# ShengkaiWu/IoU-aware-single-stage-object-detector

Hardware: AMD Instinct MI355X
Metric: images/sec at 1333x800, IoU-aware RetinaNet R-50-FPN (higher is better)
Workload: dtype fp32; 1 GPU; IoU-aware RetinaNet R-50-FPN fp32, batch 8 per GPU, 3x800x1344 (1333x800 padded to /32), random-init weights, whole inference path incl. NMS, device-to-host copy and bbox2result (the reference's simple_test: per-class arrays on the host; batch i's host part runs under batch i+1's device part, the last one inside the timed region); global_batch=8, parallelism=dp1, dets_per_image=100

## Files before the change

### include/iouaware.h

```cpp
#ifndef IOUAWARE_H
#define IOUAWARE_H

#include <stddef.h>
#include <stdint.h>

#ifdef __cplusplus
extern "C" {
#endif

#define IA_MAX_LEVELS 8
#define IA_MAX_ANCHORS 16
#define IA_MAX_NMS_PRE 4096
#define IA_MAX_CANDIDATES 8192
#define IA_MAX_PER_IMG 1024

#define IA_F32 0
#define IA_BF16 1
#define IA_F16 2
#define IA_F64 3

#define IA_LAYOUT_NCHW 0
#define IA_LAYOUT_NHWC 1

#define IA_CLS_SIGMOID 0
// ... 88 lines not shown
                           int batch, int R, int C, float score_thr, float iou_thr,
                           int max_per_img, int candidates, void *workspace,
                           size_t workspace_bytes, float *dets, int32_t *labels, int32_t *rows,
                           int32_t *num, void *stream);

int ia_decode_stage(const ia_head_geom *g, const ia_level_ptrs *p, int batch, int dtype,
                    const float *img_hw, const float *scale_factor, int rescale, void *workspace,
                    size_t workspace_bytes, void *stream);

int ia_get_bboxes_workspace_layout(const ia_head_geom *g, int batch, size_t offsets[8]);

size_t ia_nms_workspace_bytes(int n);
int ia_nms(const float *dets, int n, float iou_thr, int32_t *keep, int32_t *count, void *workspace,
           size_t workspace_bytes, void *stream);

size_t ia_nms_f64_workspace_bytes(int n);
int ia_nms_f64(const double *dets, int n, float iou_thr, int32_t *keep, int32_t *count,
               void *workspace, size_t workspace_bytes, void *stream);

int ia_soft_nms(const float *dets, int n, float iou_thr, int method, float sigma, float min_score,
                float *out_dets, int32_t *out_inds, int32_t *count, void *stream);

typedef struct {
    const uint8_t *src;
    int32_t src_h, src_w, dst_h, dst_w, flip;
} ia_image_desc;
int ia_image_transform(const ia_image_desc *imgs, int batch, const float *mean, const float *std,
                       int to_rgb, int pad_h, int pad_w, int channels_last, float *out,
                       void *stream);

typedef struct {
    int32_t num_levels, batch;
    int32_t H[IA_MAX_LEVELS], W[IA_MAX_LEVELS];
} ia_wino_geom;
typedef struct {
    int32_t c0, n;
    int32_t dst_channels, dst_offset;
    float *dst[IA_MAX_LEVELS];
} ia_wino_seg;
int ia_wino_tiles(const ia_wino_geom *g, int32_t *tiles);
int ia_wino_input_transform(const ia_wino_geom *g, const float *const *x, int channels, int groups,
                            const float *pre_scale, const float *pre_shift, int pre_relu, float *V,
                            void *stream);
int ia_wino_output_transform(const ia_wino_geom *g, const float *M, int channels, int groups,
                             const float *bias, int relu, int nseg, const ia_wino_seg *segs,
                             void *stream);
int ia_wino_mid_transform(const ia_wino_geom *g, const float *M, int channels, int groups_m,
                          const float *bias, int relu, float *V, int groups_v, void *stream);
int ia_wino_in_gemm(const ia_wino_geom *g, const float *const *x, int channels, const float *pre_scale,
                    const float *pre_shift, int pre_relu, const float *u_packed, float *M, void *stream);
int ia_wino_conv3x3_c64(const ia_wino_geom *g, const float *const *x, int channels, const float *pre_scale,
                        const float *pre_shift, int pre_relu, const float *u_packed, const float *bias,
                        int relu, float *const *y, void *stream);

int ia_wino_grad_output_transform(const ia_wino_geom *g, const float *const *dy, int channels,
                                  float *dM, void *stream);

#define IA_COLSUM_MAX_STRIPS 512
size_t ia_relu_bwd_bias_grad_workspace_bytes(int64_t rows, int n);
int ia_wino_weight_transform(const float *w, int n_in, int n_out, int64_t stride_in,
                             int64_t stride_out, int64_t stride_ky, int64_t stride_kx, int flip,
                             const double *G, float *U, void *stream);
int ia_wino_weight_grad(const float *dU, int n_in, int n_out, const double *G, float *dW,
                        int64_t stride_in, int64_t stride_out, int64_t stride_ky, int64_t stride_kx,
                        void *stream);
int ia_bn_fold_fwd(const float *w, const float *gamma, const float *beta, const float *mean,
                   const float *inv_std, int cout, int K, float *w_out, float *b_out, void *stream);
int ia_bn_fold_bwd(const float *dw_folded, const float *db_folded, const float *w, const float *gamma,
                   const float *mean, const float *inv_std, int cout, int K, float *dw,
                   float *dgamma, float *dbeta, void *stream);
int ia_relu_bwd_bias_grad(const float *dy, const float *y, int64_t rows, int n, float *g, float *db,
                          void *workspace, size_t workspace_bytes, void *stream);

int ia_linear_bias_act(const float *A, const float *W, const float *bias, const float *residual,
                       float *D, int64_t rows, int k, int n, int relu, void *workspace,
                       size_t workspace_bytes, void *stream);
int ia_linear_bias_act_bf16(const void *A, const void *W, const float *bias, const void *residual,
                            void *D, int64_t rows, int k, int n, int relu, void *workspace,
                            size_t workspace_bytes, void *stream);
int ia_batched_gemm(const float *A, const float *W, float *D, int batch, int64_t rows, int k, int n,
                    void *workspace, size_t workspace_bytes, void *stream);
int ia_batched_gemm_stream(const float *A, const float *W, float *D, int batch, int64_t rows, int k,
                           int n, void *stream);

size_t ia_im2col3x3_bytes(int B, int H, int W, int C, int stride, int dtype);
int ia_im2col3x3_nhwc(const void *x, void *col, int B, int H, int W, int C, int stride, int dtype,
                      void *stream);
int ia_conv1x1_strided(const void *x, const void *W_kn, const float *bias, const void *residual,
                       void *D, int B, int H, int W, int k, int n, int stride, int relu, int dtype,
                       void *workspace, size_t workspace_bytes, void *stream);
int ia_col2im3x3_nhwc(const void *dcol, void *dx, int B, int H, int W, int C, int stride, int dtype,
                      void *stream);

size_t ia_deform_im2col3x3_bytes(int B, int H, int W, int C, int stride, int pad, int dil);
int ia_deform_im2col3x3_nhwc(const float *x, const float *offset, int64_t offset_pix_stride,
                             const float *mask, int64_t mask_pix_stride, int mask_logits,
                             float *col, int B, int H, int W, int C, int stride, int pad,
                             int dil, int deformable_groups, void *stream);
int ia_deform_col2im3x3_nhwc(const float *dcol, const float *x, const float *offset,
                             int64_t offset_pix_stride, const float *mask,
                             int64_t mask_pix_stride, float *dx, float *d_offset, float *d_mask,
                             int B, int H, int W, int C, int stride, int pad, int dil,
                             int deformable_groups, void *stream);

int ia_gemm_tuning(int mode);

// ... 416 lines not shown
```

### iou-aware-single-stage-object-detector_amd/csrc/wino.hip

```cpp
#include <string.h>
#include "ia_internal.hpp"
#include "ia_wino.hpp"

namespace ia {

typedef float f32x4_t __attribute__((ext_vector_type(4)));
__device__ __forceinline__ float4 load_nt(const float *p)
{
    const f32x4_t q = __builtin_nontemporal_load(reinterpret_cast<const f32x4_t *>(p));
    return make_float4(q.x, q.y, q.z, q.w);
}
__device__ __forceinline__ void store_nt(float *p, const float4 &v)
{
    f32x4_t q; q.x = v.x; q.y = v.y; q.z = v.z; q.w = v.w;
    __builtin_nontemporal_store(q, reinterpret_cast<f32x4_t *>(p));
}
__device__ __forceinline__ float4 f4(float v) { return make_float4(v, v, v, v); }
__device__ __forceinline__ float4 operator+(const float4 &a, const float4 &b) { return make_float4(a.x + b.x, a.y + b.y, a.z + b.z, a.w + b.w); }
__device__ __forceinline__ float4 operator-(const float4 &a, const float4 &b) { return make_float4(a.x - b.x, a.y - b.y, a.z - b.z, a.w - b.w); }
__device__ __forceinline__ float4 operator*(float s, const float4 &a) { return make_float4(s * a.x, s * a.y, s * a.z, s * a.w); }

__device__ __forceinline__ void bt6(const float4 (&d)[6], float4 (&o)[6])
{
    o[0] = (4.0f * d[0] - 5.0f * d[2]) + d[4];
// ... 559 lines not shown
#pragma unroll
            for (int i = 0; i < 4; ++i) {
                float4 o[4];
                at6(s[i], o);
                const int y = 4 * tyi + i, ly = ly0 + i;
#pragma unroll
                for (int j = 0; j < 4; ++j) {
                    const int xx = 4 * txi + j, lx = lx0 + j;
                    float4 v = o[j] + bz;
                    if (a.relu) v = make_float4(v.x > 0.f ? v.x : 0.f, v.y > 0.f ? v.y : 0.f,
                                                v.z > 0.f ? v.z : 0.f, v.w > 0.f ? v.w : 0.f);
                    v = (y < H && xx < W) ? v : f4(0.0f);
                    if (ly >= 0 && ly < kMidP && lx >= 0 && lx < kMidP)
                        *reinterpret_cast<float4 *>(sy + (ly * kMidP + lx) * kMidCh) = v;
                }
            }
        } else {
#pragma unroll
            for (int i = 0; i < 4; ++i)
#pragma unroll
                for (int j = 0; j < 4; ++j) {
                    const int ly = ly0 + i, lx = lx0 + j;
                    if (ly >= 0 && ly < kMidP && lx >= 0 && lx < kMidP)
                        *reinterpret_cast<float4 *>(sy + (ly * kMidP + lx) * kMidCh) = f4(0.0f);
                }
        }
    }
    __syncthreads();

    const int tl = tid / kMidQ, tyl = tl / kMidB, txl = tl - tyl * kMidB;
    const int tyi = kMidB * byi + tyl, txi = kMidB * bxi + txl;
    if (tyi >= ty_n || txi >= tx) return;
    const float *sp = s_y + ((4 * tyl) * kMidP + 4 * txl) * kMidCh + cq;
    float4 tmp[6][6];
#pragma unroll
    for (int j = 0; j < 6; ++j) {
        float4 col[6], o[6];
#pragma unroll
        for (int i = 0; i < 6; ++i) col[i] = *reinterpret_cast<const float4 *>(sp + (i * kMidP + j) * kMidCh);
        bt6(col, o);
#pragma unroll
        for (int i = 0; i < 6; ++i) tmp[i][j] = o[i];
        __builtin_amdgcn_sched_barrier(0);
    }
    float *v = a.V + (size_t)gv * 36 * vstride + (size_t)(tbase + tyi * tx + txi) * a.Cv + (c - gv * a.Cv);
#pragma unroll
    for (int i = 0; i < 6; ++i) {
        float4 o[6];
        bt6(tmp[i], o);
#pragma unroll
        for (int j = 0; j < 6; ++j)
            *reinterpret_cast<float4 *>(v + (size_t)(i * 6 + j) * vstride) = o[j];
    }
}

}

extern "C" {

int ia_wino_tiles(const ia_wino_geom *g, int32_t *tiles)
{
    ia::WinoLevels w;
    int rc = ia::make_wino_levels(g, w);
    if (rc) return rc;
    if (tiles) *tiles = w.tile_off[w.L];
    return 0;
}

int ia_wino_input_transform(const ia_wino_geom *g, const float *const *x, int channels, int groups,
                            const float *pre_scale, const float *pre_shift, int pre_relu, float *V,
                            void *stream)
{
    ia::WinoInArgs a;
    int rc = ia::make_wino_levels(g, a.lv);
    if (rc) return rc;
    if (!x || !V || channels < 4 || (channels & 3) || groups < 1 || channels % groups) return IA_E_ARG;
    a.Ctot = channels; a.Cg = channels / groups; a.T = a.lv.tile_off[a.lv.L];
    if (a.Cg & 3) return IA_E_ARG;
    for (int l = 0; l < IA_MAX_LEVELS; ++l) {
        a.x[l] = (l < a.lv.L) ? x[l] : nullptr;
        if (l < a.lv.L && (!x[l] || ((uintptr_t)x[l] & 15u))) return IA_E_ARG;
    }
    a.V = V;
    if (pre_scale && !pre_shift) return IA_E_ARG;
    a.pre_scale = pre_scale; a.pre_shift = pre_shift; a.pre_relu = pre_relu ? 1 : 0;
    a.tpw = ia::tiles_per_wave(channels);
    const int waves = (a.T + a.tpw - 1) / a.tpw;
    dim3 grid((unsigned)((waves + 7) / 8 * 8), (unsigned)((channels / 4 + 63) / 64));
    if (a.tpw > 1) hipLaunchKernelGGL(ia::k_wino_in<true>, grid, dim3(64), 0, (hipStream_t)stream, a);
    else hipLaunchKernelGGL(ia::k_wino_in<false>, grid, dim3(64), 0, (hipStream_t)stream, a);
    return ia::hip_status(hipGetLastError());
}

int ia_wino_in_gemm(const ia_wino_geom *g, const float *const *x, int channels, const float *pre_scale,
                    const float *pre_shift, int pre_relu, const float *u_packed, float *M, void *stream)
{
    ia::WinoInGemmArgs a;
    int rc = ia::make_wino_levels(g, a.lv);
    if (rc) return rc;
    if (!x || !u_packed || !M || channels != 64) return IA_E_ARG;
    if (((uintptr_t)u_packed & 15u) || ((uintptr_t)M & 15u) || ((uintptr_t)pre_scale & 15u) ||
        ((uintptr_t)pre_shift & 15u))
        return IA_E_ARG;
    for (int l = 0; l < IA_MAX_LEVELS; ++l) {
        a.x[l] = (l < a.lv.L) ? x[l] : nullptr;
        if (l < a.lv.L && (!x[l] || ((uintptr_t)x[l] & 15u))) return IA_E_ARG;
// ... 73 lines not shown
    a.T = a.lv.tile_off[a.lv.L]; a.relu = relu ? 1 : 0; a.nseg = nseg;
    memset(a.seg, 0, sizeof(a.seg));
    for (int k = 0; k < nseg; ++k) {
        const ia_wino_seg &s = segs[k];
        if (s.c0 < 0 || s.n < 1 || s.c0 + s.n > channels || s.dst_channels < s.n + s.dst_offset ||
            s.dst_offset < 0)
            return IA_E_ARG;
        if (k > 0 && s.c0 < segs[k - 1].c0 + segs[k - 1].n) return IA_E_ARG;
        a.seg[k].c0 = s.c0; a.seg[k].n = s.n; a.seg[k].Cdst = s.dst_channels; a.seg[k].coff = s.dst_offset;
        for (int l = 0; l < a.lv.L; ++l) {
            if (!s.dst[l]) return IA_E_ARG;
            a.seg[k].dst[l] = s.dst[l];
        }
    }
    a.tpw = ia::tiles_per_wave(channels);
    const int waves = (a.T + a.tpw - 1) / a.tpw;
    dim3 grid((unsigned)((waves + 7) / 8 * 8), (unsigned)((channels / 4 + 63) / 64));
    if (a.tpw > 1) hipLaunchKernelGGL(ia::k_wino_out<true>, grid, dim3(64), 0, (hipStream_t)stream, a);
    else hipLaunchKernelGGL(ia::k_wino_out<false>, grid, dim3(64), 0, (hipStream_t)stream, a);
    return ia::hip_status(hipGetLastError());
}

int ia_wino_mid_transform(const ia_wino_geom *g, const float *M, int channels, int groups_m,
                          const float *bias, int relu, float *V, int groups_v, void *stream)
{
    ia::WinoMidArgs a;
    int rc = ia::make_wino_levels(g, a.lv);
    if (rc) return rc;
    if (!M || !V || channels < ia::kMidCh || groups_m < 1 || channels % groups_m || groups_v < 1 ||
        channels % groups_v)
        return IA_E_ARG;
    a.M = M; a.bias = bias; a.V = V; a.Ctot = channels;
    a.Cm = channels / groups_m; a.Cv = channels / groups_v;
    if (a.Cm % ia::kMidCh || a.Cv % ia::kMidCh || ((uintptr_t)M & 15u) || ((uintptr_t)V & 15u) ||
        ((uintptr_t)bias & 15u))
        return IA_E_ARG;
    a.T = a.lv.tile_off[a.lv.L]; a.relu = relu ? 1 : 0;
    int64_t n = 0;
    for (int l = 0; l < IA_MAX_LEVELS; ++l) {
        const bool on = l < a.lv.L;
        const int ty = on ? a.lv.tpi[l] / a.lv.tx[l] : 0;
        a.bx[l] = on ? (a.lv.tx[l] + ia::kMidB - 1) / ia::kMidB : 0;
        a.bpi[l] = on ? ((ty + ia::kMidB - 1) / ia::kMidB) * a.bx[l] : 0;
        a.blk_off[l] = (int32_t)n;
        n += (int64_t)a.lv.B * a.bpi[l];
    }
    a.blk_off[IA_MAX_LEVELS] = (int32_t)n;
    a.nblk = (int32_t)n;
    dim3 grid((unsigned)((n + 7) / 8 * 8), (unsigned)(channels / ia::kMidCh));
    hipLaunchKernelGGL(ia::k_wino_mid, grid, dim3(ia::kMidThreads), 0, (hipStream_t)stream, a);
    return ia::hip_status(hipGetLastError());
}

}
```

### iou-aware-single-stage-object-detector_amd/iouaware/_lib.py

```python
import ctypes as C
import os

IA_MAX_LEVELS = 8
IA_MAX_ANCHORS = 16
IA_MAX_NMS_PRE = 4096
IA_MAX_CANDIDATES = 8192
IA_MAX_PER_IMG = 1024
IA_F32, IA_BF16, IA_F16, IA_F64 = 0, 1, 2, 3
IA_LAYOUT_NCHW, IA_LAYOUT_NHWC = 0, 1
IA_CLS_SIGMOID, IA_CLS_SOFTMAX = 0, 1
IA_CLS_SIGMOID_NOIOU, IA_CLS_SOFTMAX_NOIOU = 2, 3
IA_LOSS_SLOTS = 64
IA_MAX_TARGET_BATCH = 16
IA_GN_CHUNK = 256

_CSRC = os.path.join(os.path.dirname(os.path.abspath(__file__)), '..', 'csrc')
SO_PATH = os.path.abspath(os.path.join(_CSRC, 'libiouaware_hip.so'))


class HeadGeom(C.Structure):
    _fields_ = [('num_levels', C.c_int32), ('num_anchors', C.c_int32),
                ('num_classes', C.c_int32), ('nms_pre', C.c_int32),
                ('H', C.c_int32 * IA_MAX_LEVELS), ('W', C.c_int32 * IA_MAX_LEVELS),
                ('stride', C.c_int32 * IA_MAX_LEVELS),
# ... 105 lines not shown
SIGNATURES = {
    'ia_version': (C.c_char_p, []),
    'ia_geom_sizes': (_i, [_G, C.POINTER(C.c_int32), C.POINTER(C.c_int32), C.POINTER(C.c_int32)]),
    'ia_decode_fuse_rowmax': (_i, [_G, _P, _i, _i, _vp, _vp]),
    'ia_select_topk_workspace_bytes': (_sz, [_G, _i]),
    'ia_select_topk': (_i, [_G, _vp, _i, _vp, _vp, _sz, _vp]),
    'ia_decode_fuse_rowmax_grouped': (_i, [_G, _P, _i, _i, _vp, _vp, _sz, _vp]),
    'ia_select_topk_grouped': (_i, [_G, _vp, _i, _vp, _vp, _sz, _vp]),
    'ia_decode_stage': (_i, [_G, _P, _i, _i, _vp, _vp, _i, _vp, _sz, _vp]),
    'ia_get_bboxes_status_offset': (_sz, [_G, _i]),
    'ia_debug_fused_spin_limit': (_i, [_i64]),
    'ia_profile_stage_events': (_i, [_vp, _vp]),
    'ia_gather_decode': (_i, [_G, _P, _i, _i, _vp, _vp, _vp, _i, _vp, _vp, _vp, _vp]),
    'ia_multiclass_nms_workspace_bytes': (_sz, [_i, _i, _i]),
    'ia_multiclass_nms': (_i, [_vp, _vp, _vp, _i, _i, _i, _f, _f, _i, _vp, _sz, _vp, _vp, _vp,
                               _vp, _vp, _vp, _vp]),
    'ia_multiclass_soft_nms_workspace_bytes': (_sz, [_i, _i, _i]),
    'ia_multiclass_soft_nms': (_i, [_vp, _vp, _i, _i, _i, _f, _f, _i, _f, _f, _i, _vp, _sz, _vp, _vp,
                                    _vp, _vp, _vp, _vp, _vp]),
    'ia_soft_nms': (_i, [_vp, _i, _f, _i, _f, _f, _vp, _vp, _vp, _vp]),
    'ia_get_bboxes_workspace_bytes': (_sz, [_G, _i]),
    'ia_get_bboxes': (_i, [_G, _P, _i, _i, _vp, _vp, _i, _f, _f, _i, _vp, _sz, _vp, _vp, _vp,
                           _vp, _vp]),
    'ia_multiclass_nms_lazy_workspace_bytes': (_sz, [_i, _i, _i]),
    'ia_multiclass_nms_lazy': (_i, [_vp, _vp, _vp, _i, _i, _i, _f, _f, _i, _i, _vp, _sz, _vp, _vp, _vp,
                                    _vp, _vp]),
    'ia_get_bboxes_lazy': (_i, [_G, _P, _i, _i, _vp, _vp, _i, _f, _f, _i, _i, _vp, _sz, _vp, _vp, _vp,
                                _vp, _vp]),
    'ia_get_bboxes_workspace_layout': (_i, [_G, _i, C.POINTER(_sz * 8)]),
    'ia_nms_workspace_bytes': (_sz, [_i]),
    'ia_nms': (_i, [_vp, _i, _f, _vp, _vp, _vp, _sz, _vp]),
    'ia_nms_f64_workspace_bytes': (_sz, [_i]),
    'ia_nms_f64': (_i, [_vp, _i, _f, _vp, _vp, _vp, _sz, _vp]),
    'ia_image_transform': (_i, [C.POINTER(ImageDesc), _i, C.POINTER(C.c_float), C.POINTER(C.c_float),
                                _i, _i, _i, _i, _vp, _vp]),
    'ia_wino_tiles': (_i, [C.POINTER(WinoGeom), C.POINTER(C.c_int32)]),
    'ia_wino_input_transform': (_i, [C.POINTER(WinoGeom), C.POINTER(C.c_void_p), _i, _i, _vp, _vp, _i,
                                     _vp, _vp]),
    'ia_wino_grad_output_transform': (_i, [C.POINTER(WinoGeom), C.POINTER(C.c_void_p), _i, _vp, _vp]),
    'ia_wino_weight_transform': (_i, [_vp, _i, _i, C.c_int64, C.c_int64, C.c_int64, C.c_int64, _i,
                                      C.POINTER(C.c_double), _vp, _vp]),
    'ia_wino_weight_grad': (_i, [_vp, _i, _i, C.POINTER(C.c_double), _vp, C.c_int64, C.c_int64,
                                 C.c_int64, C.c_int64, _vp]),
    'ia_bn_fold_fwd': (_i, [_vp, _vp, _vp, _vp, _vp, _i, _i, _vp, _vp, _vp]),
    'ia_bn_fold_bwd': (_i, [_vp, _vp, _vp, _vp, _vp, _vp, _i, _i, _vp, _vp, _vp, _vp]),
    'ia_relu_bwd_bias_grad_workspace_bytes': (C.c_size_t, [C.c_int64, _i]),
    'ia_relu_bwd_bias_grad': (_i, [_vp, _vp, C.c_int64, _i, _vp, _vp, _vp, C.c_size_t, _vp]),
    'ia_wino_output_transform': (_i, [C.POINTER(WinoGeom), _vp, _i, _i, _vp, _i, _i,
                                      C.POINTER(WinoSeg), _vp]),
    'ia_wino_mid_transform': (_i, [C.POINTER(WinoGeom), _vp, _i, _i, _vp, _i, _vp, _i, _vp]),
    'ia_wino_in_gemm': (_i, [C.POINTER(WinoGeom), C.POINTER(C.c_void_p), _i, _vp, _vp, _i, _vp, _vp, _vp]),
    'ia_wino_conv3x3_c64': (_i, [C.POINTER(WinoGeom), C.POINTER(C.c_void_p), _i, _vp, _vp, _i, _vp, _vp, _i,
                                 C.POINTER(C.c_void_p), _vp]),
    'ia_linear_bias_act': (_i, [_vp, _vp, _vp, _vp, _vp, _i64, _i, _i, _i, _vp, _sz, _vp]),
    'ia_linear_bias_act_bf16': (_i, [_vp, _vp, _vp, _vp, _vp, _i64, _i, _i, _i, _vp, _sz, _vp]),
    'ia_batched_gemm': (_i, [_vp, _vp, _vp, _i, _i64, _i, _i, _vp, _sz, _vp]),
    'ia_batched_gemm_stream': (_i, [_vp, _vp, _vp, _i, _i64, _i, _i, _vp]),
    'ia_linear_bias_act_wt': (_i, [_vp, _vp, _vp, _vp, _vp, _i64, _i, _i, _i, _vp, _sz, _vp]),
    'ia_gemm_tuning': (_i, [_i]),
    'ia_im2col3x3_bytes': (_sz, [_i, _i, _i, _i, _i, _i]),
    'ia_im2col3x3_nhwc': (_i, [_vp, _vp, _i, _i, _i, _i, _i, _i, _vp]),
    'ia_col2im3x3_nhwc': (_i, [_vp, _vp, _i, _i, _i, _i, _i, _i, _vp]),
    'ia_deform_im2col3x3_bytes': (_sz, [_i, _i, _i, _i, _i, _i, _i]),
    'ia_deform_im2col3x3_nhwc': (_i, [_vp, _vp, _i64, _vp, _i64, _i, _vp, _i, _i, _i, _i, _i, _i, _i, _i, _vp]),
    'ia_deform_col2im3x3_nhwc': (_i, [_vp, _vp, _vp, _i64, _vp, _i64, _vp, _vp, _vp, _i, _i, _i, _i, _i, _i,
                                      _i, _i, _vp]),
    'ia_conv1x1_strided': (_i, [_vp, _vp, _vp, _vp, _vp, _i, _i, _i, _i, _i, _i, _i, _i, _vp, _sz, _vp]),
    'ia_gemm_table_add': (_i, [_i64, _i64, _i64, _i, _i, _i, _i]),
    'ia_gemm_table_clear': (_i, []),
    'ia_gemm_table_dump': (_i, [_vp, _i]),
    'ia_gemm_table_stats': (_i, [_vp]),
    'ia_gemm_library_version': (_i, []),
    'ia_gemm_tn': (_i, [_vp, _vp, _vp, _i, _i64, _i, _i, _vp, _sz, _vp]),
    'ia_focal_loss_fwd': (_i, [_vp, _i, _vp, _vp, _i, _i, _i, _i, _f, _f, _vp, _vp]),
    'ia_focal_loss_bwd': (_i, [_vp, _i, _vp, _vp, _i, _i, _i, _i, _f, _f, _f, _vp, _vp, _vp]),
    'ia_smooth_l1_fwd': (_i, [_vp, _i, _vp, _vp, _i, _i, _i, _f, _vp, _vp]),
    'ia_smooth_l1_bwd': (_i, [_vp, _i, _vp, _vp, _i, _i, _i, _f, _f, _vp, _vp, _vp]),
    'ia_balanced_l1_fwd': (_i, [_vp, _i, _vp, _vp, _i, _i, _i, _f, _f, _f, _vp, _vp]),
    'ia_balanced_l1_bwd': (_i, [_vp, _i, _vp, _vp, _i, _i, _i, _f, _f, _f, _f, _vp, _vp, _vp]),
    'ia_focal_loss_balanced_fwd': (_i, [_vp, _i, _vp, _vp, _vp, _i, _i, _i, _i, _f, _f, _f, _vp, _vp]),
    'ia_focal_loss_balanced_bwd': (_i, [_vp, _i, _vp, _vp, _vp, _i, _i, _i, _i, _f, _f, _f, _vp, _f,
                                        _vp, _vp, _vp]),
    'ia_smooth_l1_balanced_fwd': (_i, [_vp, _i, _vp, _vp, _vp, _i, _i, _i, _f, _f, _vp, _vp]),
    'ia_smooth_l1_balanced_bwd': (_i, [_vp, _i, _vp, _vp, _vp, _i, _i, _i, _f, _f, _f, _vp, _vp,
                                       _vp]),
    'ia_iou_bce_fwd': (_i, [_G, _i, _vp, _vp, _i, _vp, _vp, _i, _vp, _vp, _vp]),
    'ia_iou_bce_bwd': (_i, [_G, _i, _vp, _vp, _i, _vp, _vp, _i, _f, _vp, _vp, _vp, _vp]),
    'ia_anchor_targets': (_i, [_G, _vp, _vp, _vp, _i, _i, _vp, _f, _f, _f, _f, _vp, _vp, _vp, _vp,
                               _vp, _vp, _vp]),
    'ia_anchor_targets_ptrs': (_i, [_G, C.POINTER(C.c_void_p), C.POINTER(C.c_void_p),
                                    C.POINTER(C.c_int32), _i, C.POINTER(C.c_int32), _f, _f, _f, _f,
                                    _vp, _vp, _vp, _vp, _vp, _vp, _vp]),
    'ia_head_loss_workspace_bytes': (_sz, [_G, _i]),
    'ia_head_loss_workspace_bytes_cfg': (_sz, [_G, _i, C.POINTER(HeadLossCfg)]),
    'ia_head_loss_fwd': (_i, [_G, _P, _i, _i, C.POINTER(HeadTargets), C.POINTER(HeadLossCfg), _vp,
                              _sz, _vp, _vp]),
    'ia_head_loss_bwd': (_i, [_G, _P, _i, _i, C.POINTER(HeadTargets), C.POINTER(HeadLossCfg), _vp,
                              _vp, _vp, _P, _vp]),
    'ia_head_loss_fwd_nhwc': (_i, [_G, _P, C.POINTER(LevelPixStrides), _i, C.POINTER(HeadTargets),
                                   C.POINTER(HeadLossCfg), _vp, _sz, _vp, _vp]),
    'ia_head_loss_bwd_nhwc': (_i, [_G, _P, C.POINTER(LevelPixStrides), _i, C.POINTER(HeadTargets),
                                   C.POINTER(HeadLossCfg), _vp, _vp, _P, C.POINTER(LevelPixStrides),
                                   _vp]),
    'ia_head_loss_fwd_box': (_i, [_G, _P, _i, _i, C.POINTER(HeadTargets), C.POINTER(HeadLossCfg),
                                  C.POINTER(BoxLossCfg), _vp, _sz, _vp, _vp]),
    'ia_head_loss_bwd_box': (_i, [_G, _P, _i, _i, C.POINTER(HeadTargets), C.POINTER(HeadLossCfg),
# ... 140 lines not shown
```

### iou-aware-single-stage-object-detector_amd/iouaware/fuse.py

```python
import types

import torch
import torch.nn.functional as F
from torch.nn.modules.batchnorm import _BatchNorm

from . import ops, train_fuse
from .backbones import BasicBlock, Bottleneck, ResNet
from .deform_conv import _DeformBase, _one
from .layers import ConvModule, Scale
from .winograd import plain_3x3

_VEC = {torch.float32: 4, torch.bfloat16: 8}


def _fold_bn(bn):
    if not isinstance(bn, _BatchNorm):
        raise TypeError('only BatchNorm can be folded, got %s' % type(bn).__name__)
    with torch.no_grad():
        var, mean = bn.running_var.float(), bn.running_mean.float()
        g = bn.weight.float() if bn.weight is not None else torch.ones_like(var)
        b = bn.bias.float() if bn.bias is not None else torch.zeros_like(var)
        scale = g / torch.sqrt(var + bn.eps)
        shift = b - mean * scale
    return scale.contiguous(), shift.contiguous()


def _stamp_slots(module):
    slots, links = [], []
    tops = ('conv1', module.norm1_name) if isinstance(module, ResNet) else (None,)
    for top_name in tops:
        top = module if top_name is None else module._modules[top_name]
        if top_name is not None:
            links.append((module._modules, top_name, top))
        stack = [top]
        while stack:
            m = stack.pop()
            for name, child in m._modules.items():
                if child is not None:
                    links.append((m._modules, name, child))
                    stack.append(child)
            if isinstance(m, torch.nn.Conv2d):
                slots.append((m._parameters, 'weight'))
                if m.bias is not None:
                    slots.append((m._parameters, 'bias'))
            elif isinstance(m, _BatchNorm) and m.running_var is not None:
                slots.append((m._buffers, 'running_var'))
                if m.weight is not None:
                    slots.append((m._parameters, 'weight'))
            elif isinstance(m, torch.nn.GroupNorm) and m.weight is not None:
                slots.append((m._parameters, 'weight'))
                slots.append((m._parameters, 'bias'))
            elif isinstance(m, Scale):
                slots.append((m._parameters, 'scale'))
            elif isinstance(m, _DeformBase):
                slots.append((m._parameters, 'weight'))
    return slots, links


def _stamp(module):
# ... 56 lines not shown
    else:
        om = co(out).contiguous(memory_format=torch.channels_last)
    n = 18 * self.deformable_groups
    return ops.deform_conv3x3(out, om[:, :n], om[:, n:] if self.with_modulated_dcn else None, f['dcn2'],
                              f['b2'], _one(c2.stride, 'stride'), _one(c2.padding, 'padding'),
                              _one(c2.dilation, 'dilation'), self.deformable_groups, relu=True,
                              mask_logits=True)


def _bottleneck_run(self, x, h1=None, nxt=None):
    if not _fast(self, x):
        if _train(self) and train_fuse.bottleneck_usable(self, x):
            return train_fuse.bottleneck_forward(self, x), None
        return type(self).forward(self, x), None
    f = self._ia_fused
    lt = 'w1' in f and x.dtype in (torch.float32, torch.bfloat16) \
        and x.is_contiguous(memory_format=torch.channels_last)
    if h1 is not None:
        w, out, pre = f, h1, None
    elif lt:
        w = _weights_for(f, x.dtype)
        out, pre = ops.linear_bias_act(x, w['w1'], f['b1'], relu=True), None
    else:
        out, pre = self.conv1(x), (f['s1'], f['b1'], True)
    gw = f.get('gconv2')
    wino = f.get('wino2')
    if getattr(self, 'with_dcn', False):
        if pre is not None:
            out = ops.channel_affine_act_(out, f['s1'], f['b1'], relu=True)
        out = _dcn_conv2(self, f, out)
    elif gw is not None and out.dtype == torch.float32 \
            and out.is_contiguous(memory_format=torch.channels_last):
        if pre is not None:
            out = ops.channel_affine_act_(out, f['s1'], f['b1'], relu=True)
        out = ops.grouped_conv3x3(out, gw, f['b2'], self.conv2.groups, self.conv2.stride[0],
                                  relu=True)
    elif gw is not None and out.dtype == torch.bfloat16 and self.conv2.in_channels % 32 == 0 \
            and out.is_contiguous(memory_format=torch.channels_last) and self._ia_gconv_bf16:
        if pre is not None:
            out = ops.channel_affine_act_(out, f['s1'], f['b1'], relu=True)
        wp = f.get('_gconv2_bf16')
        if wp is None:
            wp = f['_gconv2_bf16'] = ops.pack_grouped_weight_bf16(self.conv2.weight, f['s2'])
        out = ops.grouped_conv3x3_bf16(out, wp, f['b2'], self.conv2.groups, self.conv2.stride[0],
                                       relu=True)
    elif wino is not None and wino.usable(out):
        out = wino(out, pre=pre)
    elif pre is None and 'c3' in f and out.dtype == torch.bfloat16 \
            and out.is_contiguous(memory_format=torch.channels_last):
        wp = f.get('_c3_packed')
        if wp is None:
            wp = f['_c3_packed'] = ops.conv3x3_bf16_pack(f['c3'])
        out = ops.conv3x3_bf16(out, wp, f['b2'], self.conv2.out_channels, relu=True)
    elif lt and 'im2col2' in f and out.is_contiguous(memory_format=torch.channels_last):
        out = ops.conv3x3_im2col(out, w['im2col2'], f['b2'], stride=self.conv2.stride[0], relu=True)
    else:
        if pre is not None:
            out = ops.channel_affine_act_(out, f['s1'], f['b1'], relu=True)
        out = ops.channel_affine_act_(self.conv2(out), f['s2'], f['b2'], relu=True)
    if lt and out.is_contiguous(memory_format=torch.channels_last):
        if self.downsample is None:
            if nxt is not None:
                return ops.conv1x1_chain(out, w['w3'], f['b3'], x, nxt['w1'], nxt['b1'])
            return ops.linear_bias_act(out, w['w3'], f['b3'], residual=x, relu=True), None
        if 'wd' in f:
            idn = ops.linear_bias_act(x, w['wd'], f['b3d'])
            if nxt is not None:
                return ops.conv1x1_chain(out, w['w3'], None, idn, nxt['w1'], nxt['b1'])
            return ops.linear_bias_act(out, w['w3'], None, residual=idn, relu=True), None
        ds = self.downsample[0]
        if 'wd_s' in f:
            idn = ops.conv1x1_strided(x, w['wd_s'], None, None, stride=ds.stride[0])
        else:
            idn = F.conv2d(x, w['wd_conv'], None, ds.stride, ds.padding)
        return ops.linear_bias_act(out, w['w3'], f['b3d'], residual=idn, relu=True), None
    out = self.conv3(out)
    if self.downsample is None:
        return ops.channel_affine_act_(out, f['s3'], f['b3'], residual=x, relu=True), None
    idn = self.downsample[0](x)
    return ops.channel_affine_act_(out, f['s3'], f['b3'], residual=idn, res_scale=f['sd'],
                                   res_shift=f['bd'], relu=True), None


def _chain_ok(blk, nxt, x):
    f, g = getattr(blk, '_ia_fused', None), getattr(nxt, '_ia_fused', None)
    if f is None or g is None or 'w3' not in f or 'w1' not in g or nxt.downsample is not None:
        return False
    if getattr(blk, 'with_dcn', False) or getattr(nxt, 'with_dcn', False):
        return False
    if blk.downsample is not None and 'wd' not in f:
        return False
    k, n = f['w3'].shape
    return tuple(g['w1'].shape) == (n, g['w1'].shape[1]) and ops.chain_usable(x, k, n, g['w1'].shape[1]) \
        and x.is_contiguous(memory_format=torch.channels_last)


def _has_hooks(m):
    import torch.nn.modules.module as tm
    return bool(m._forward_hooks or m._forward_pre_hooks or tm._global_forward_hooks
                or tm._global_forward_pre_hooks)


def _layer_forward(self, x):
    blocks = list(self)
    if not all(isinstance(b, Bottleneck) and hasattr(b, '_ia_opts') for b in blocks) or not blocks:
        return torch.nn.Sequential.forward(self, x)
# ... 229 lines not shown
        m._ia_wino = WinogradHead(m)
        m._ia_c3 = None
    elif type(m).__name__ in ('IoUawareFCOSHead', 'FCOSHead'):
        from .winograd import WinogradFCOSHead
        m._ia_wino = WinogradFCOSHead(m)
        m._ia_c3 = None
    elif isinstance(m, Bottleneck):
        f = {}
        f['s1'], f['b1'] = _fold_bn(m.norm1)
        f['s2'], f['b2'] = _fold_bn(m.norm2)
        f['s3'], f['b3'] = _fold_bn(m.norm3)
        if m.downsample is not None:
            f['sd'], f['bd'] = _fold_bn(m.downsample[1])
        if winograd and _gemm_ok(m.conv1) and _gemm_ok(m.conv3):
            with torch.no_grad():
                def kn(conv, scale):
                    w = conv.weight.float().view(conv.out_channels, conv.in_channels)
                    return (w * scale.view(-1, 1)).t().contiguous()
                f['w1'], f['w3'] = kn(m.conv1, f['s1']), kn(m.conv3, f['s3'])
                if m.downsample is not None:
                    ds = m.downsample[0]
                    f['b3d'] = (f['b3'] + f['bd']).contiguous()
                    if _gemm_ok(ds):
                        f['wd'] = kn(ds, f['sd'])
                    elif tuple(ds.kernel_size) == (1, 1) and tuple(ds.padding) == (0, 0) \
                            and ds.groups == 1 and ds.bias is None and ds.stride[0] == ds.stride[1]:
                        f['wd_s'] = kn(ds, f['sd'])
                    else:
                        f['wd_conv'] = (ds.weight.float() * f['sd'].view(-1, 1, 1, 1)).contiguous(
                            memory_format=torch.channels_last)
        c2 = m.conv2
        dcn = getattr(m, 'with_dcn', False)
        if dcn and winograd and 'w1' in f and c2.in_channels % (4 * m.deformable_groups) == 0 \
                and c2.groups == 1 and tuple(c2.kernel_size) == (3, 3) and c2.weight.dtype == torch.float32:
            co = m.conv2_offset
            f['dcn2'] = ops.conv3x3_weight_kn(c2.weight, f['s2'])
            if _im2col_ok(co):
                f['off_im2col'] = ops.conv3x3_weight_kn(co.weight)
                f['off_b'] = None if co.bias is None else co.bias.detach().float().contiguous()
            elif _wino_ok(co):
                from .winograd import WinogradConv3x3
                f['off_wino'] = WinogradConv3x3(co.weight, co.bias, relu=False)
        if dcn:
            pass
        elif winograd and c2.groups > 1 and tuple(c2.kernel_size) == (3, 3) \
                and tuple(c2.padding) == (1, 1) and tuple(c2.dilation) == (1, 1) \
                and c2.stride[0] == c2.stride[1] and c2.stride[0] in (1, 2) and c2.bias is None \
                and c2.in_channels == c2.out_channels \
                and c2.in_channels // c2.groups in (4, 8, 16, 32) \
                and c2.in_channels % (32 if c2.in_channels // c2.groups == 32 else 16) == 0:
            f['gconv2'] = ops.pack_grouped_weight(c2.weight, f['s2'])
        if not dcn and winograd and _im2col_ok(c2) and c2.bias is None and 'w1' in f:
            f['im2col2'] = ops.conv3x3_weight_kn(c2.weight, f['s2'])
        if not dcn and winograd and _wino_ok(m.conv2) and m.conv2.bias is None:
            from .winograd import WinogradConv3x3
            with torch.no_grad():
                w2 = m.conv2.weight.float() * f['s2'].view(-1, 1, 1, 1)
            f['wino2'] = WinogradConv3x3(w2, f['b2'], relu=True)
            if m.conv2.in_channels % 32 == 0 and m.conv2.out_channels % 2 == 0 \
                    and getattr(m.conv2, 'padding_mode', 'zeros') == 'zeros':
                f['c3'] = w2
        m._ia_fused = f
    elif isinstance(m, BasicBlock):
        f = {}
        f['s1'], f['b1'] = _fold_bn(m.norm1)
        f['s2'], f['b2'] = _fold_bn(m.norm2)
        if m.downsample is not None:
            f['sd'], f['bd'] = _fold_bn(m.downsample[1])
        m._ia_fused = f
    elif isinstance(m, ResNet):
        f = {}
        f['s'], f['b'] = _fold_bn(m.norm1)
        mp = m.maxpool
        f['pool'] = (_pair(mp.kernel_size), _pair(mp.stride), _pair(mp.padding),
                     _pair(mp.dilation), mp.ceil_mode) == ((3, 3), (2, 2), (1, 1), (1, 1), False)
        c1 = m.conv1
        if winograd and isinstance(c1, torch.nn.Conv2d) and tuple(c1.weight.shape) == (64, 3, 7, 7) \
                and tuple(c1.stride) == (2, 2) and tuple(c1.padding) == (3, 3) and tuple(c1.dilation) == (1, 1) \
                and c1.groups == 1 and c1.bias is None and getattr(c1, 'padding_mode', 'zeros') == 'zeros':
            f['stem_w'] = ops.stem_weight(c1.weight)
        m._ia_fused = f
    elif isinstance(m, ConvModule):
        f = {}
        c = m.conv
        if m.with_norm:
            if not isinstance(m.norm, _BatchNorm):
                return False
            f['s'], f['b'] = _fold_bn(m.norm)
            if c.bias is not None:
                with torch.no_grad():
                    f['b'] = (f['b'] + c.bias.detach().float() * f['s']).contiguous()
        elif c.bias is not None:
            f['bias'] = c.bias.detach().float().contiguous()
        if winograd and tuple(c.kernel_size) == (1, 1) and tuple(c.stride) == (1, 1) \
                and tuple(c.padding) == (0, 0) and c.groups == 1:
            with torch.no_grad():
                w = c.weight.float().view(c.out_channels, c.in_channels)
                if m.with_norm:
                    f['w_kn'], f['b_kn'] = (w * f['s'].view(-1, 1)).t().contiguous(), f['b']
                else:
                    f['w_kn'] = w.t().contiguous()
                    f['b_kn'] = None if c.bias is None else c.bias.detach().float().contiguous()
        if winograd and not m.with_norm and _im2col_ok(c):
            f['im2col'] = ops.conv3x3_weight_kn(c.weight)
        if winograd and fpn_conv and not m.with_norm and _wino_ok(m.conv):
            from .winograd import WinogradConv3x3
# ... 88 lines not shown
```

### iou-aware-single-stage-object-detector_amd/iouaware/winograd.py

```python
import collections
import ctypes as C

import numpy as np
import torch

from . import _lib
from .ops import _ptr, _stream, stream_id

_G = np.array([[1 / 4, 0, 0], [-1 / 6, -1 / 6, -1 / 6], [-1 / 6, 1 / 6, -1 / 6],
               [1 / 24, 1 / 12, 1 / 6], [1 / 24, -1 / 12, 1 / 6], [0, 0, 1]], dtype=np.float64)


_G_DEV = {}


def transform_weight(w):
    if w.dim() != 4 or w.shape[2] != 3 or w.shape[3] != 3:
        raise ValueError('Winograd F(4,3) needs a 3x3 kernel, got %s' % (tuple(w.shape),))
    g = w.detach().to(torch.float64)
    G = _G_DEV.get(g.device)
    if G is None:
        G = _G_DEV[g.device] = torch.from_numpy(_G).to(g.device)
    u = torch.einsum('ik,ockl,jl->ijco', G, g, G)
    return u.reshape(36, g.shape[1], g.shape[0]).to(torch.float32).contiguous()
# ... 160 lines not shown
    if epilogue is not None:
        bias, relu, ys = epilogue
        if out is not None or len(ys) != len(xs):
            raise ValueError('the one-launch form writes ys, one per level, and no M')
        yptrs = (C.c_void_p * len(ys))(*[y.data_ptr() for y in ys])
        _lib.check(_lib.lib().ia_wino_conv3x3_c64(C.byref(plan.geom), ptrs, int(xs[0].shape[1]), _ptr(ps),
                                                  _ptr(pb), int(bool(pr)), _ptr(u_packed), _ptr(bias),
                                                  int(bool(relu)), yptrs, _stream()),
                   'ia_wino_conv3x3_c64')
        return ys
    _lib.check(_lib.lib().ia_wino_in_gemm(C.byref(plan.geom), ptrs, int(xs[0].shape[1]), _ptr(ps), _ptr(pb),
                                          int(bool(pr)), _ptr(u_packed), _ptr(out), _stream()),
               'ia_wino_in_gemm')
    return out


class WinogradConv3x3(object):

    def __init__(self, weight, bias, relu=False):
        self.u = transform_weight(weight)
        self.u_packed = None
        if self.u.shape[1] == self.u.shape[2] and self.u.shape[1] in _IN_GEMM_CHANNELS:
            self.u_packed = pack_u_fragments(self.u)
        self.bias = None if bias is None else bias.detach().to(torch.float32).contiguous()
        self.relu = relu
        self.cin, self.cout = self.u.shape[1], self.u.shape[2]
        if self.cout % 4:
            raise ValueError('output channels must be a multiple of 4')
        self._plans = collections.OrderedDict()

    def usable(self, x):
        return _usable(x) and x.shape[1] == self.cin \
            and not (torch.is_grad_enabled() and x.requires_grad)

    def __call__(self, x, pre=None):
        key = (x.shape[0], tuple(x.shape[-2:]), x.device, stream_id())
        plan = _plan_for(self._plans, key, lambda: _Plan([tuple(x.shape[-2:])], x.shape[0], x.device))
        if (FUSE_IN_GEMM and self.u_packed is not None and STREAM_BMM
                and (self.cin, self.cout) in _STREAM_BMM_SHAPES and plan.T >= 4096
                and x.dtype == torch.float32):
            if FUSE_OUT:
                y = torch.empty((x.shape[0], self.cout) + tuple(x.shape[-2:]), dtype=torch.float32,
                                device=x.device, memory_format=torch.channels_last)
                input_transform_gemm(plan, [x], self.u_packed, None, pre, epilogue=(self.bias, self.relu, [y]))
                return y
            m = input_transform_gemm(plan, [x], self.u_packed, plan.buf('m', (36, plan.T, self.cout)), pre)
        else:
            v = input_transform(plan, [x], 1, plan.buf('v', (36, plan.T, self.cin)), pre)
            m = batched_gemm(v, self.u, plan.buf('m', (36, plan.T, self.cout)))
        y = torch.empty((x.shape[0], self.cout) + tuple(x.shape[-2:]), dtype=torch.float32,
                        device=x.device, memory_format=torch.channels_last)
        output_transform(plan, m, self.cout, 1, self.bias, self.relu, [(0, self.cout, [y], 0)])
        return y


def plain_3x3(conv):
    return (tuple(conv.kernel_size) == (3, 3) and tuple(conv.stride) == (1, 1)
            and tuple(conv.padding) == (1, 1) and tuple(conv.dilation) == (1, 1) and conv.groups == 1)


def _pair(a, b, F, granule):
    na, nb = a.out_channels, (0 if b is None else b.out_channels)
    n_pad = (na + nb + granule - 1) // granule * granule
    dev = a.weight.device
    u = torch.zeros((36, F, n_pad), dtype=torch.float32, device=dev)
    u[:, :, :na] = transform_weight(a.weight)
    bias = torch.zeros(n_pad, dtype=torch.float32, device=dev)
    bias[:na] = a.bias.detach().float()
    if b is not None:
        u[:, :, na:na + nb] = transform_weight(b.weight)
        bias[na:na + nb] = b.bias.detach().float()
    return u.contiguous(), bias.contiguous(), na, nb


class _WinogradTowers(object):

    FUSE_MID = True
    mid_bias = None

    def __init__(self, head):
        convs_c, convs_r = list(head.cls_convs), list(head.reg_convs)
        self.n_layers = len(convs_c)
        F = head.feat_channels
        if head.in_channels % 4 or F % 4:
            raise ValueError('channel counts must be multiples of 4')
        self.F, self.cin = F, head.in_channels
        self.u0 = torch.cat([transform_weight(convs_c[0].conv.weight),
                             transform_weight(convs_r[0].conv.weight)], dim=2).contiguous()
        self.u = [torch.cat([transform_weight(convs_c[i].conv.weight),
                             transform_weight(convs_r[i].conv.weight)], dim=0).contiguous()
                  for i in range(1, self.n_layers)]
        self._plans = collections.OrderedDict()

    def usable(self, feats):
        return all(_usable(x) and x.shape[1] == self.cin for x in feats) \
            and not torch.is_grad_enabled()

    def _towers(self, feats):
        B, dev = feats[0].shape[0], feats[0].device
        sizes = [tuple(x.shape[-2:]) for x in feats]
        key = (B, tuple(sizes), dev, stream_id())
        plan = _plan_for(self._plans, key, lambda: _Plan(sizes, B, dev))
        T, F = plan.T, self.F
        v = input_transform(plan, feats, 1, plan.buf('v', (36, T, self.cin)))
        m = batched_gemm(v, self.u0, plan.buf('m', (36, T, 2 * F)))
        new = lambda c: [torch.empty((B, c, h, w), dtype=torch.float32, device=dev,
# ... 118 lines not shown
```

Before: 417.5 img/s.

## Add Winograd F(4,2) phase-split path for stride-2 3x3 bottleneck convs

Adds a Winograd path for the stride-2 3x3 convs in the ResNet bottlenecks. The input is split into four polyphase components, so each one becomes a 2x2 stride-1 conv, which is then handled with F(4,2) transforms (5x5 tiles) and a batched GEMM over 25 points with a 4x-wide K dimension. The goal is to cut the multiplies and im2col traffic of the stride-2 convs at channels 128/256/512. The cost is two new transform kernels, transform buffers, and some fp32 numerical error from the larger-ratio Winograd transform.

```diff
diff --git a/include/iouaware.h b/include/iouaware.h
--- a/include/iouaware.h
+++ b/include/iouaware.h
@@ -164,6 +164,10 @@
 int ia_wino_conv3x3_c64(const ia_wino_geom *g, const float *const *x, int channels, const float *pre_scale,
                         const float *pre_shift, int pre_relu, const float *u_packed, const float *bias,
                         int relu, float *const *y, void *stream);
+int ia_wino_s2_input_transform(const float *x, int batch, int H, int W, int channels, float *V,
+                               void *stream);
+int ia_wino_s2_output_transform(const float *M, int batch, int Ho, int Wo, int channels,
+                                const float *bias, int relu, float *y, void *stream);
 
 int ia_wino_grad_output_transform(const ia_wino_geom *g, const float *const *dy, int channels,
                                   float *dM, void *stream);
diff --git a/iou-aware-single-stage-object-detector_amd/csrc/wino.hip b/iou-aware-single-stage-object-detector_amd/csrc/wino.hip
--- a/iou-aware-single-stage-object-detector_amd/csrc/wino.hip
+++ b/iou-aware-single-stage-object-detector_amd/csrc/wino.hip
@@ -635,6 +635,146 @@
         for (int j = 0; j < 6; ++j)
             *reinterpret_cast<float4 *>(v + (size_t)(i * 6 + j) * vstride) = o[j];
     }
+}
+
+__device__ __forceinline__ void bt5(const float4 (&d)[5], float4 (&o)[5])
+{
+    o[0] = 0.5f * (d[0] - d[2]) + (d[3] - d[1]);
+    o[1] = 0.5f * (d[2] - d[1]) + d[3];
+    o[2] = (0.5f * d[1] - 1.5f * d[2]) + d[3];
+    o[3] = d[3] - d[1];
+    o[4] = 0.5f * (d[1] - d[3]) + (d[4] - d[2]);
+}
+
+__device__ __forceinline__ void at5(const float4 (&m)[5], float4 (&o)[4])
+{
+    const float4 s12 = m[1] + m[2], d12 = m[1] - m[2];
+    o[0] = (m[0] + s12) + m[3];
+    o[1] = d12 + 0.5f * m[3];
+    o[2] = s12 + 0.25f * m[3];
+    o[3] = (d12 + 0.125f * m[3]) + m[4];
+}
+
+struct WinoS2InArgs {
+    WinoLevels lv;
+    const float *x;
+    float *V;
+    int32_t H, W, C, T, tpw;
+};
+
+template <bool PACKED>
+__global__ void __launch_bounds__(64) k_wino_s2_in(WinoS2InArgs a)
+{
+    const int Cv = 4 * a.C;
+    const LaneMap lm = lane_map<PACKED>(Cv, a.T, a.tpw);
+    if (!lm.on) return;
+    const int t = lm.t;
+    const TileRef r = locate_tile(a.lv, t);
+    const int phase = lm.c / a.C, c = lm.c - phase * a.C;
+    const int H = a.H, W = a.W;
+    const int yb = 2 * r.y0 - 2 + (phase >> 1), xb = 2 * r.x0 - 2 + (phase & 1);
+    const float *x = a.x + (size_t)r.b * H * W * a.C + c;
+    float4 d[5][5];
+#pragma unroll
+    for (int i = 0; i < 5; ++i) {
+        const int y = yb + 2 * i;
+        const int yc = (y >= 0 && y < H) ? y : 0;
+#pragma unroll
+        for (int j = 0; j < 5; ++j) {
+            const int xx = xb + 2 * j;
+            const int xc = (xx >= 0 && xx < W) ? xx : 0;
+            d[i][j] = *reinterpret_cast<const float4 *>(x + ((size_t)yc * W + xc) * a.C);
+        }
+    }
+#pragma unroll
+    for (int i = 0; i < 5; ++i) {
+        const int y = yb + 2 * i;
+        const bool yin = (y >= 0) && (y < H);
+#pragma unroll
+        for (int j = 0; j < 5; ++j) {
+            const int xx = xb + 2 * j;
+            const bool in = yin && (xx >= 0) && (xx < W);
+            d[i][j] = in ? d[i][j] : f4(0.0f);
+        }
+    }
+    float4 tmp[5][5];
+#pragma unroll
+    for (int j = 0; j < 5; ++j) {
+        float4 col[5], o[5];
+#pragma unroll
+        for (int i = 0; i < 5; ++i) col[i] = d[i][j];
+        bt5(col, o);
+#pragma unroll
+        for (int i = 0; i < 5; ++i) tmp[i][j] = o[i];
+    }
+    float *v = a.V + (size_t)t * Cv + lm.c;
+    const size_t kstride = (size_t)a.T * Cv;
+#pragma unroll
+    for (int i = 0; i < 5; ++i) {
+        float4 o[5];
+        bt5(tmp[i], o);
+#pragma unroll
+        for (int j = 0; j < 5; ++j)
+            *reinterpret_cast<float4 *>(v + (size_t)(i * 5 + j) * kstride) = o[j];
+    }
+}
+
+struct WinoS2OutArgs {
+    WinoLevels lv;
+    const float *M;
+    const float *bias;
+    float *y;
+    int32_t N, T, relu, tpw;
+};
+
+template <bool PACKED>
+__global__ void __launch_bounds__(64) k_wino_s2_out(WinoS2OutArgs a)
+{
+    const LaneMap lm = lane_map<PACKED>(a.N, a.T, a.tpw);
+    if (!lm.on) return;
+    const int t = lm.t, c = lm.c;
+    int H, W;
+    const TileRef r = locate_tile(a.lv, t, &H, &W);
+    const float *m = a.M + (size_t)t * a.N + c;
+    const size_t kstride = (size_t)a.T * a.N;
+    float4 bz = f4(0.0f);
+    if (a.bias) bz = *reinterpret_cast<const float4 *>(a.bias + c);
+    float4 s[4][5];
+#pragma unroll
+    for (int j = 0; j < 5; ++j) {
+        float4 col[5], o[4];
+#pragma unroll
+        for (int i = 0; i < 5; ++i) col[i] = load_nt(m + (size_t)(i * 5 + j) * kstride);
+        at5(col, o);
+#pragma unroll
+        for (int i = 0; i < 4; ++i) s[i][j] = o[i];
+    }
+    float *const dst = a.y + c;
+#pragma unroll
+    for (int i = 0; i < 4; ++i) {
+        float4 o[4];
+        at5(s[i], o);
+        const int y = r.y0 + i;
+#pragma unroll
+        for (int j = 0; j < 4; ++j) {
+            const int xx = r.x0 + j;
+            if (y >= H || xx >= W) continue;
+            float4 v = o[j] + bz;
+            if (a.relu) v = make_float4(v.x > 0.f ? v.x : 0.f, v.y > 0.f ? v.y : 0.f,
+                                        v.z > 0.f ? v.z : 0.f, v.w > 0.f ? v.w : 0.f);
+            const size_t pix = ((size_t)r.b * H + y) * W + xx;
+            *reinterpret_cast<float4 *>(dst + pix * a.N) = v;
+        }
+    }
+}
+
+static int make_s2_levels(int batch, int Ho, int Wo, WinoLevels &w)
+{
+    if (batch < 1 || Ho < 1 || Wo < 1) return IA_E_ARG;
+    ia_wino_geom g;
+    memset(&g, 0, sizeof(g));
+    g.num_levels = 1; g.batch = batch; g.H[0] = Ho; g.W[0] = Wo;
+    return make_wino_levels(&g, w);
 }
 
 }
@@ -814,4 +954,39 @@
     return ia::hip_status(hipGetLastError());
 }
 
-}
+int ia_wino_s2_input_transform(const float *x, int batch, int H, int W, int channels, float *V,
+                               void *stream)
+{
+    ia::WinoS2InArgs a;
+    if (H < 1 || W < 1) return IA_E_ARG;
+    int rc = ia::make_s2_levels(batch, (H - 1) / 2 + 1, (W - 1) / 2 + 1, a.lv);
+    if (rc) return rc;
+    if (!x || !V || channels < 4 || (channels & 3) || channels > (1 << 20)) return IA_E_ARG;
+    if (((uintptr_t)x & 15u) || ((uintptr_t)V & 15u)) return IA_E_ARG;
+    a.x = x; a.V = V; a.H = H; a.W = W; a.C = channels; a.T = a.lv.tile_off[1];
+    a.tpw = ia::tiles_per_wave(4 * channels);
+    const int waves = (a.T + a.tpw - 1) / a.tpw;
+    dim3 grid((unsigned)((waves + 7) / 8 * 8), (unsigned)((channels + 63) / 64));
+    if (a.tpw > 1) hipLaunchKernelGGL(ia::k_wino_s2_in<true>, grid, dim3(64), 0, (hipStream_t)stream, a);
+    else hipLaunchKernelGGL(ia::k_wino_s2_in<false>, grid, dim3(64), 0, (hipStream_t)stream, a);
+    return ia::hip_status(hipGetLastError());
+}
+
+int ia_wino_s2_output_transform(const float *M, int batch, int Ho, int Wo, int channels,
+                                const float *bias, int relu, float *y, void *stream)
+{
+    ia::WinoS2OutArgs a;
+    int rc = ia::make_s2_levels(batch, Ho, Wo, a.lv);
+    if (rc) return rc;
+    if (!M || !y || channels < 4 || (channels & 3)) return IA_E_ARG;
+    if (((uintptr_t)M & 15u) || ((uintptr_t)y & 15u) || ((uintptr_t)bias & 15u)) return IA_E_ARG;
+    a.M = M; a.bias = bias; a.y = y; a.N = channels; a.T = a.lv.tile_off[1]; a.relu = relu ? 1 : 0;
+    a.tpw = ia::tiles_per_wave(channels);
+    const int waves = (a.T + a.tpw - 1) / a.tpw;
+    dim3 grid((unsigned)((waves + 7) / 8 * 8), (unsigned)((channels / 4 + 63) / 64));
+    if (a.tpw > 1) hipLaunchKernelGGL(ia::k_wino_s2_out<true>, grid, dim3(64), 0, (hipStream_t)stream, a);
+    else hipLaunchKernelGGL(ia::k_wino_s2_out<false>, grid, dim3(64), 0, (hipStream_t)stream, a);
+    return ia::hip_status(hipGetLastError());
+}
+
+}
diff --git a/iou-aware-single-stage-object-detector_amd/iouaware/_lib.py b/iou-aware-single-stage-object-detector_amd/iouaware/_lib.py
--- a/iou-aware-single-stage-object-detector_amd/iouaware/_lib.py
+++ b/iou-aware-single-stage-object-detector_amd/iouaware/_lib.py
@@ -181,6 +181,8 @@
     'ia_wino_in_gemm': (_i, [C.POINTER(WinoGeom), C.POINTER(C.c_void_p), _i, _vp, _vp, _i, _vp, _vp, _vp]),
     'ia_wino_conv3x3_c64': (_i, [C.POINTER(WinoGeom), C.POINTER(C.c_void_p), _i, _vp, _vp, _i, _vp, _vp, _i,
                                  C.POINTER(C.c_void_p), _vp]),
+    'ia_wino_s2_input_transform': (_i, [_vp, _i, _i, _i, _i, _vp, _vp]),
+    'ia_wino_s2_output_transform': (_i, [_vp, _i, _i, _i, _i, _vp, _i, _vp, _vp]),
     'ia_linear_bias_act': (_i, [_vp, _vp, _vp, _vp, _vp, _i64, _i, _i, _i, _vp, _sz, _vp]),
     'ia_linear_bias_act_bf16': (_i, [_vp, _vp, _vp, _vp, _vp, _i64, _i, _i, _i, _vp, _sz, _vp]),
     'ia_batched_gemm': (_i, [_vp, _vp, _vp, _i, _i64, _i, _i, _vp, _sz, _vp]),
diff --git a/iou-aware-single-stage-object-detector_amd/iouaware/fuse.py b/iou-aware-single-stage-object-detector_amd/iouaware/fuse.py
--- a/iou-aware-single-stage-object-detector_amd/iouaware/fuse.py
+++ b/iou-aware-single-stage-object-detector_amd/iouaware/fuse.py
@@ -4,7 +4,7 @@
 import torch.nn.functional as F
 from torch.nn.modules.batchnorm import _BatchNorm
 
-from . import ops, train_fuse
+from . import ops, train_fuse, winograd
 from .backbones import BasicBlock, Bottleneck, ResNet
 from .deform_conv import _DeformBase, _one
 from .layers import ConvModule, Scale
@@ -167,6 +167,9 @@
         if wp is None:
             wp = f['_c3_packed'] = ops.conv3x3_bf16_pack(f['c3'])
         out = ops.conv3x3_bf16(out, wp, f['b2'], self.conv2.out_channels, relu=True)
+    elif lt and 'wino_s2' in f and winograd.STRIDE2 and out.dtype == torch.float32 \
+            and self.conv2.in_channels in winograd.S2_CHANNELS and f['wino_s2'].usable(out):
+        out = f['wino_s2'](out)
     elif lt and 'im2col2' in f and out.is_contiguous(memory_format=torch.channels_last):
         out = ops.conv3x3_im2col(out, w['im2col2'], f['b2'], stride=self.conv2.stride[0], relu=True)
     else:
@@ -502,6 +505,9 @@
             f['gconv2'] = ops.pack_grouped_weight(c2.weight, f['s2'])
         if not dcn and winograd and _im2col_ok(c2) and c2.bias is None and 'w1' in f:
             f['im2col2'] = ops.conv3x3_weight_kn(c2.weight, f['s2'])
+            if c2.stride[0] == 2 and c2.out_channels % 4 == 0 and c2.weight.dtype == torch.float32:
+                from .winograd import WinogradConv3x3S2
+                f['wino_s2'] = WinogradConv3x3S2(c2.weight, f['s2'], f['b2'], relu=True)
         if not dcn and winograd and _wino_ok(m.conv2) and m.conv2.bias is None:
             from .winograd import WinogradConv3x3
             with torch.no_grad():
diff --git a/iou-aware-single-stage-object-detector_amd/iouaware/winograd.py b/iou-aware-single-stage-object-detector_amd/iouaware/winograd.py
--- a/iou-aware-single-stage-object-detector_amd/iouaware/winograd.py
+++ b/iou-aware-single-stage-object-detector_amd/iouaware/winograd.py
@@ -236,6 +236,82 @@
                         device=x.device, memory_format=torch.channels_last)
         output_transform(plan, m, self.cout, 1, self.bias, self.relu, [(0, self.cout, [y], 0)])
         return y
+
+
+STRIDE2 = True
+S2_CHANNELS = (128, 256, 512)
+
+_G2 = np.array([[2, 0], [1, 1], [-1 / 3, 1 / 3], [-8 / 3, -4 / 3], [0, 1]], dtype=np.float64)
+_S2_TAPS = {1: (0, 2), 0: (None, 1)}
+
+
+def phase_kernels_s2(w, scale=None):
+    if w.dim() != 4 or w.shape[2] != 3 or w.shape[3] != 3:
+        raise ValueError('Winograd F(4,2) on the phase split needs a 3x3 kernel, got %s' % (tuple(w.shape),))
+    g = w.detach().to(torch.float64)
+    if scale is not None:
+        g = g * scale.detach().to(torch.float64).view(-1, 1, 1, 1)
+    out = torch.zeros((4,) + tuple(g.shape[:2]) + (2, 2), dtype=torch.float64, device=g.device)
+    for r in (0, 1):
+        for c in (0, 1):
+            for a, ky in enumerate(_S2_TAPS[r]):
+                for b, kx in enumerate(_S2_TAPS[c]):
+                    if ky is not None and kx is not None:
+                        out[2 * r + c, :, :, a, b] = g[:, :, ky, kx]
+    return out
+
+
+def transform_weight_s2(w, scale=None):
+    g = phase_kernels_s2(w, scale)
+    G = torch.from_numpy(_G2).to(g.device)
+    u = torch.einsum('ia,pocab,jb->ijpco', G, g, G)
+    return u.reshape(25, 4 * g.shape[2], g.shape[1]).to(torch.float32).contiguous()
+
+
+def s2_out_hw(H, W):
+    return (int(H) - 1) // 2 + 1, (int(W) - 1) // 2 + 1
+
+
+def s2_input_transform(plan, x, out):
+    B, ch, H, W = x.shape
+    _lib.check(_lib.lib().ia_wino_s2_input_transform(_ptr(x), int(B), int(H), int(W), int(ch), _ptr(out),
+                                                     _stream()), 'ia_wino_s2_input_transform')
+    return out
+
+
+def s2_output_transform(plan, m, bias, relu, y):
+    B, n, Ho, Wo = y.shape
+    _lib.check(_lib.lib().ia_wino_s2_output_transform(_ptr(m), int(B), int(Ho), int(Wo), int(n), _ptr(bias),
+                                                      int(bool(relu)), _ptr(y), _stream()),
+               'ia_wino_s2_output_transform')
+    return y
+
+
+class WinogradConv3x3S2(object):
+
+    def __init__(self, weight, scale=None, bias=None, relu=False):
+        self.u = transform_weight_s2(weight, scale)
+        self.bias = None if bias is None else bias.detach().to(torch.float32).contiguous()
+        self.relu = relu
+        self.cin, self.cout = self.u.shape[1] // 4, self.u.shape[2]
+        if self.cin % 4 or self.cout % 4:
+            raise ValueError('channel counts must be multiples of 4')
+        self._plans = collections.OrderedDict()
+
+    def usable(self, x):
+        return _usable(x) and x.shape[1] == self.cin \
+            and not (torch.is_grad_enabled() and x.requires_grad)
+
+    def __call__(self, x):
+        B, _, H, W = x.shape
+        Ho, Wo = s2_out_hw(H, W)
+        key = (B, (H, W), x.device, stream_id())
+        plan = _plan_for(self._plans, key, lambda: _Plan([(Ho, Wo)], B, x.device))
+        v = s2_input_transform(plan, x, plan.buf('v', (25, plan.T, 4 * self.cin)))
+        m = batched_gemm(v, self.u, plan.buf('m', (25, plan.T, self.cout)))
+        y = torch.empty((B, self.cout, Ho, Wo), dtype=torch.float32, device=x.device,
+                        memory_format=torch.channels_last)
+        return s2_output_transform(plan, m, self.bias, self.relu, y)
 
 
 def plain_3x3(conv):
```

Result: no change. 420.8 img/s (median of 6 runs) (+0.8%).
